# apcamargo/genomad

Hardware: NVIDIA H100
Metric: nn_classification_windows_per_s (higher is better)
Workload: dtype split operands on wgmma (conv: fp16 main pass + two e4m3 correction passes; w_v: 3 fp16 passes), fp32 accumulate; fp32-equivalent (<=1e-4 vs the fp32 oracle, measured ~1e-5)

## Files before the change

genomad_b200/csrc/api.cu:

```cuda
#include <cuda.h>
#include <cuda_runtime.h>
#include <cuda_fp16.h>

#include <algorithm>
#include <cmath>
#include <cstdio>
#include <cstring>
#include <string>
#include <vector>

#include "../../include/gnm.h"
#include "common.cuh"
#include "encode.cuh"
#include "conv_t.cuh"
#include "layer1_wv.cuh"
#include "conv_ref.cuh"
#include "igloo.cuh"
#include "dense.cuh"
#include "logits_tc.cuh"
#include "wv_gather.cuh"
#include "contigs.cuh"
#include "attr.cuh"
#include "neighbours.cuh"
#include "clusters.cuh"
// ... 36 lines not shown
  float* conv1_table = nullptr; float* conv1_triple = nullptr; float* conv1_bias = nullptr;
  uint8_t* wpack[4] = {nullptr, nullptr, nullptr, nullptr};
  float conv_out_scale[2] = {1.f, 1.f};
  float* conv_bias[2] = {nullptr, nullptr};
  float* conv_w32[2] = {nullptr, nullptr};
  float* wv32[2] = {nullptr, nullptr};
  float* ent_w[2] = {nullptr, nullptr}; int32_t* ent_pos[2] = {nullptr, nullptr}; int32_t* slot_of[2] = {nullptr, nullptr};
  float* wbias[2] = {nullptr, nullptr}; float* wqk[2] = {nullptr, nullptr};
  float* d0w = nullptr; float* d0b = nullptr; float* bn0_scale = nullptr; float* bn0_shift = nullptr;
  float* d1w = nullptr; float* d1b = nullptr; float* bn1_scale = nullptr; float* bn1_shift = nullptr;
  float* d2w = nullptr; float* d2b = nullptr;
  float* dwT_hi[2] = {nullptr, nullptr}; float* dwT_lo[2] = {nullptr, nullptr};
  float* hA_hi[2] = {nullptr, nullptr}; float* hA_lo[2] = {nullptr, nullptr};
  CUtensorMap tm_hd_a[2][2]; CUtensorMap tm_hd_b[2][2];
  uint8_t* ybuf[2] = {nullptr, nullptr};
  int ybuf_fp8lo[2] = {0, 0};
  float* q[2] = {nullptr, nullptr};
  float* mpi[2] = {nullptr, nullptr};
  float* mpi_hi[2] = {nullptr, nullptr}; float* mpi_lo[2] = {nullptr, nullptr};
  float* wqkT_hi[2] = {nullptr, nullptr}; float* wqkT_lo[2] = {nullptr, nullptr};
  CUtensorMap tm_lg_a[2][2];
  CUtensorMap tm_lg_b[2][2];
  float* part = nullptr;
  int2* grp[2] = {nullptr, nullptr};
  int32_t* band_gstart[2] = {nullptr, nullptr};
  uint4* wfrag[2] = {nullptr, nullptr};
  float gather_unscale[2] = {1.f, 1.f};
  float wv_out_scale[2] = {1.f, 1.f};
  std::vector<int32_t> band_groups[2];
  int32_t* cta_split = nullptr;
  std::vector<int32_t> split_host[2];
  int split_groups[2] = {-1, -1}, split_grid[2] = {-1, -1};
  float wv_cost_base = 1.f, wv_cost_group = 0.1f;
  int mb_pad = 0;
  CUtensorMap tm_band[2];
  float* logits = nullptr; float* logits_part = nullptr; float* h0 = nullptr; float* h1 = nullptr; float* h2 = nullptr;
  float* scratch32 = nullptr;
  uint8_t* in_stage[2] = {nullptr, nullptr};
  float* out_stage[2] = {nullptr, nullptr};
  float* q_set[2][2] = {{nullptr, nullptr}, {nullptr, nullptr}};
  float* mpi_set[2][2] = {{nullptr, nullptr}, {nullptr, nullptr}};
  float* mpi_hi_set[2][2] = {{nullptr, nullptr}, {nullptr, nullptr}};
  float* mpi_lo_set[2][2] = {{nullptr, nullptr}, {nullptr, nullptr}};
  CUtensorMap tm_lg_a_set[2][2][2];
  int tail_overlap = 1;
  cudaStream_t tail_stream = nullptr;
  cudaEvent_t main_done[2] = {nullptr, nullptr}, tail_done[2] = {nullptr, nullptr};
  cudaStream_t copy_stream = nullptr, compute_stream = nullptr;
  cudaEvent_t in_ready[2] = {nullptr, nullptr}, in_free[2] = {nullptr, nullptr};
  DeviceStatus* status = nullptr;
  CUtensorMap tm_act[2];
  CUtensorMap tm_w[4];
  CUtensorMap tm_w_half[4];
  StageTimer timer;
  std::vector<void*> allocs;
  const uint8_t* attr_route[2] = {nullptr, nullptr};
// ... 114 lines not shown
      pack_stage_f8_pairs(pk, Wk + static_cast<size_t>(tap) * kC * kC, kh, std::ldexp(1.f, d), std::ldexp(1.f, S - 12 - d),
                          std::ldexp(1.f, S - 7 - d));
  return 0;
}

static constexpr int kSplitExpMin = -126, kSplitExpMax = 121;
static bool split_exponent(const float* w, size_t n, int* k) {
  float wmax = 0.f;
  for (size_t i = 0; i < n; ++i) {
    if (!std::isfinite(w[i])) return false;
    wmax = std::max(wmax, std::fabs(w[i]));
  }
  *k = 0;
  if (wmax > 0.f) { int ex; std::frexp(wmax, &ex); *k = std::max(kSplitExpMin, std::min(kSplitExpMax, 14 - ex)); }
  return true;
}

struct PatchPack {
  std::vector<float> ent_w;
  std::vector<int32_t> ent_pos, slot_of;
  std::vector<int2> groups;
  std::vector<int32_t> band_gstart;
  std::vector<uint32_t> frag;
  float unscale = 1.f;
};
static bool pack_patches(const int32_t* patches, const float* w_mult, const float* w_summer, PatchPack& o) {
  std::vector<int> order(static_cast<size_t>(kPatches) * kPatchLen);
  for (size_t i = 0; i < order.size(); ++i) order[i] = static_cast<int>(i);
  std::stable_sort(order.begin(), order.end(), [&](int a, int b) { return patches[a] < patches[b]; });
  o.ent_w.assign(static_cast<size_t>(kGsSlots) * kC, 0.f);
  o.ent_pos.assign(kGsSlots, 0);
  o.slot_of.assign(static_cast<size_t>(kPatches) * kPatchLen, 0);
  std::vector<float>& ent_w = o.ent_w;
  std::vector<int32_t>& ent_pos = o.ent_pos;
  for (size_t slot = 0; slot < order.size(); ++slot) {
    const int e = order[slot], k = e % kPatchLen;
    ent_pos[slot] = patches[e];
    o.slot_of[e] = static_cast<int32_t>(slot);
    for (int c = 0; c < kC; ++c)
      ent_w[slot * kC + c] = (w_mult[static_cast<size_t>(e) * kC + c] * w_summer[k * kC + c]) * (1.f / kActScale);
  }
  int k2;
  if (!split_exponent(ent_w.data(), ent_w.size(), &k2)) return false;
  const float wscale = std::ldexp(1.f, k2);
  o.unscale = std::ldexp(1.f, -k2);
  o.groups.clear();
  o.band_gstart.assign(kNumBands + 1, 0);
  const size_t n_ent = order.size();
  size_t slot = 0;
  for (int b = 0; b < kNumBands; ++b) {
    o.band_gstart[b] = static_cast<int32_t>(o.groups.size());
    while (slot < n_ent && ent_pos[slot] < (b + 1) * kBandRows) {
      size_t run = slot;
      while (run < n_ent && ent_pos[run] == ent_pos[slot] && run - slot < static_cast<size_t>(kWgGroupMax)) ++run;
      o.groups.push_back(make_int2(static_cast<int>(slot), (ent_pos[slot] - b * kBandRows) | (static_cast<int>(run - slot) << 8)));
      slot = run;
    }
  }
  o.band_gstart[kNumBands] = static_cast<int32_t>(o.groups.size());
  if (o.groups.empty()) o.groups.push_back(make_int2(0, 0));
  auto h2 = [](float x, float y) {
    return static_cast<uint32_t>(__half_as_ushort(__float2half_rn(x))) | (static_cast<uint32_t>(__half_as_ushort(__float2half_rn(y))) << 16);
  };
  o.frag.assign(static_cast<size_t>(kGsSlots) * 128, 0u);
  for (size_t e = 0; e < n_ent; ++e)
    for (int kh = 0; kh < 2; ++kh)
      for (int ks = 0; ks < 4; ++ks)
        for (int tig = 0; tig < 4; ++tig) {
          const int k0 = kh * 64 + ks * 16 + 2 * tig;
          const int kk[4] = {k0, k0 + 1, k0 + 8, k0 + 9};
          float hi[4], lo[4];
          for (int i = 0; i < 4; ++i) {
            const float x = ent_w[e * kC + kk[i]] * wscale;
            hi[i] = __half2float(__float2half_rn(x));
            lo[i] = x - hi[i];
          }
          uint32_t* f = &o.frag[(((e * 2 + kh) * 4 + ks) * 4 + tig) * 4];
          f[0] = h2(hi[0], hi[1]); f[1] = h2(hi[2], hi[3]); f[2] = h2(lo[0], lo[1]); f[3] = h2(lo[2], lo[3]);
        }
  return true;
}
extern "C" int gnm_pack_patches(const int32_t* patches, const float* w_mult, const float* w_summer, int32_t* slot_of, int32_t* ent_pos,
                                float* ent_w, int32_t* groups, int* n_groups, int32_t* band_first_group, uint32_t* frag, float* unscale,
                                int* layout) {
  if (layout) { layout[0] = kBandRows; layout[1] = kNumBands; layout[2] = kGsSlots; layout[3] = kWgGroupMax; }
  if (!patches && !w_mult && !w_summer) return 0;
  if (!patches || !w_mult || !w_summer || !n_groups) return fail("gnm_pack_patches: null argument");
  for (int i = 0; i < kPatches * kPatchLen; ++i)
    if (patches[i] < 0 || patches[i] >= kTok) return fail("gnm_pack_patches: patch index out of range");
  PatchPack pk;
  if (!pack_patches(patches, w_mult, w_summer, pk))
    return fail("gnm_pack_patches: folded patch weights w_mult * w_summer / 32 not finite: no fp16 operand split carries them");
  const int real_groups = pk.band_gstart[kNumBands];
  if (groups && *n_groups < real_groups) return fail("gnm_pack_patches: groups buffer too small");
  if (slot_of) std::memcpy(slot_of, pk.slot_of.data(), pk.slot_of.size() * sizeof(int32_t));
  if (ent_pos) std::memcpy(ent_pos, pk.ent_pos.data(), pk.ent_pos.size() * sizeof(int32_t));
  if (ent_w) std::memcpy(ent_w, pk.ent_w.data(), pk.ent_w.size() * sizeof(float));
  if (groups) for (int i = 0; i < real_groups; ++i) { groups[2 * i] = pk.groups[i].x; groups[2 * i + 1] = pk.groups[i].y; }
  *n_groups = real_groups;
  if (band_first_group) std::memcpy(band_first_group, pk.band_gstart.data(), pk.band_gstart.size() * sizeof(int32_t));
  if (frag) std::memcpy(frag, pk.frag.data(), pk.frag.size() * sizeof(uint32_t));
  if (unscale) *unscale = pk.unscale;
  return 0;
}

static void fold_bn(const gnm_bn_weights& b, std::vector<float>& sc, std::vector<float>& sh) {
  sc.resize(kHidden); sh.resize(kHidden);
  for (int i = 0; i < kHidden; ++i) {
// ... 58 lines not shown
      if (dev_upload(h, &h->wpack[L], pk.data(), pk.size())) return 1;
      if (dev_upload(h, &h->conv_w32[L], convw[L], static_cast<size_t>(kTaps) * kC * kC)) return 1;
    }
    for (int s = 0; s < 2; ++s) {
      int e;
      if (!split_exponent(w->igloo[s].w_v, static_cast<size_t>(kC) * kC, &e))
        return fail("gnm_create: IGLOO layer " + std::to_string(s) + ": w_v not finite: no fp16 operand split carries it");
      h->wv_out_scale[s] = std::ldexp(1.f / kActScale, -e);
      std::vector<uint8_t> pk;
      for (int kh = 0; kh < 2; ++kh)
        for (int w_lo = 0; w_lo < 2; ++w_lo) pack_stage_f16(pk, w->igloo[s].w_v, w_lo, kh, std::ldexp(1.f, e));
      if (dev_upload(h, &h->wpack[2 + s], pk.data(), pk.size())) return 1;
    }
    if (dev_upload(h, &h->conv_bias[0], w->conv2_bias, kC)) return 1;
    if (dev_upload(h, &h->conv_bias[1], w->conv3_bias, kC)) return 1;
  }
  for (int s = 0; s < 2; ++s) {
    const gnm_igloo_weights& g = w->igloo[s];
    PatchPack pk;
    if (!pack_patches(g.patches, g.w_mult, g.w_summer, pk))
      return fail("gnm_create: IGLOO layer " + std::to_string(s) +
                  ": folded patch weights w_mult * w_summer / 32 not finite: no fp16 operand split carries them");
    h->gather_unscale[s] = pk.unscale;
    h->band_groups[s].resize(kNumBands);
    for (int b = 0; b < kNumBands; ++b) h->band_groups[s][b] = pk.band_gstart[b + 1] - pk.band_gstart[b];
    if (dev_upload(h, &h->grp[s], pk.groups.data(), pk.groups.size())) return 1;
    if (dev_upload(h, &h->band_gstart[s], pk.band_gstart.data(), pk.band_gstart.size())) return 1;
    if (dev_upload(h, reinterpret_cast<uint32_t**>(&h->wfrag[s]), pk.frag.data(), pk.frag.size())) return 1;
    const std::vector<float>& ent_w = pk.ent_w;
    const std::vector<int32_t>&ent_pos = pk.ent_pos, &slot_of = pk.slot_of;
    if (dev_upload(h, &h->ent_w[s], ent_w.data(), ent_w.size())) return 1;
    if (dev_upload(h, &h->ent_pos[s], ent_pos.data(), ent_pos.size())) return 1;
    if (dev_upload(h, &h->slot_of[s], slot_of.data(), slot_of.size())) return 1;
    if (dev_upload(h, &h->wbias[s], g.w_bias, kPatches)) return 1;
    if (dev_upload(h, &h->wqk[s], g.w_qk, static_cast<size_t>(kPatches) * kPooled)) return 1;
    {
      std::vector<float> thi(static_cast<size_t>(kPooled) * kPatches), tlo(thi.size());
      for (int k = 0; k < kPatches; ++k)
        for (int n = 0; n < kPooled; ++n)
          split_tf32(g.w_qk[static_cast<size_t>(k) * kPooled + n], thi[static_cast<size_t>(n) * kPatches + k],
                     tlo[static_cast<size_t>(n) * kPatches + k]);
      if (dev_upload(h, &h->wqkT_hi[s], thi.data(), thi.size())) return 1;
      if (dev_upload(h, &h->wqkT_lo[s], tlo.data(), tlo.size())) return 1;
    }
    if (dev_upload(h, &h->wv32[s], g.w_v, static_cast<size_t>(kC) * kC)) return 1;
  }
  {
    auto bn = [&](const gnm_bn_weights& b, float** scale, float** shift) -> int {
      std::vector<float> sc, sh;
      fold_bn(b, sc, sh);
      if (dev_upload(h, scale, sc.data(), kHidden)) return 1;
// ... 172 lines not shown
  }
  conv_t_kernel<false><<<grid, kConvThreads, kConvTSmem, st>>>(h->tm_act[in_buf], h->tm_w_half[layer], p);
  return check_launch(h, "conv_t_kernel<false>");
}
static int launch_wv_tc(gnm_handle* h, int s, int buf, int n, cudaStream_t st) {
  ConvTcParams p;
  p.status = h->status;
  p.experiment = 0;
  p.dbg = nullptr;
  p.bias = nullptr; p.y_out = nullptr; p.q_out = h->q[s];
  p.out_scale = h->wv_out_scale[s];
  p.out_fp8 = 0;
  p.n_tiles = n * kUnitsPerWin;
  const int grid = std::min(h->num_sms, p.n_tiles);
  conv_t_kernel<true><<<grid, kConvThreads, kConvTSmem, st>>>(h->tm_act[buf], h->tm_w_half[2 + s], p);
  return check_launch(h, "conv_t_kernel<true>");
}

static int wv_split(gnm_handle* h, int s, int groups, int grid, cudaStream_t st) {
  if (h->split_groups[s] == groups && h->split_grid[s] == grid) return 0;
  std::vector<double> cost(kNumBands);
  double total = 0;
  for (int b = 0; b < kNumBands; ++b) {
    const int per_warp = (h->band_groups[s][b] + kWgWarps - 1) / kWgWarps;
    cost[b] = h->wv_cost_base + h->wv_cost_group * per_warp;
    total += cost[b] * groups;
  }
  std::vector<int32_t>& sp = h->split_host[s];
  sp.assign(h->num_sms + 1, kNumBands * groups);
  sp[0] = 0;
  double acc = 0;
  int c = 1;
  for (int b = 0; b < kNumBands && c < grid; ++b)
    for (int g = 0; g < groups && c < grid; ++g) {
      acc += cost[b];
      if (acc >= total * c / grid) sp[c++] = b * groups + g + 1;
    }
  for (; c <= grid; ++c) sp[c] = kNumBands * groups;
  for (int i = 1; i <= grid; ++i) sp[i] = std::max(sp[i], sp[i - 1]);
  GNM_CUDA(cudaMemcpyAsync(h->cta_split + s * (h->num_sms + 1), sp.data(), (grid + 1) * sizeof(int32_t), cudaMemcpyHostToDevice, st));
  h->split_groups[s] = groups; h->split_grid[s] = grid;
  return 0;
}

static int launch_wv_gather(gnm_handle* h, int s, int buf, int n, cudaStream_t st) {
  WvGatherParams p;
  p.q_out = h->q[s]; p.out_scale = h->wv_out_scale[s];
  p.grp = h->grp[s]; p.band_gstart = h->band_gstart[s]; p.wfrag = h->wfrag[s]; p.gather_unscale = h->gather_unscale[s]; p.part_t = h->part;
  p.n_windows = n;
  p.n_pad = (n + kBandWins - 1) / kBandWins * kBandWins;
  p.groups = p.n_pad / kBandWins;
  p.n_units = kNumBands * p.groups;
  p.status = h->status;
  p.experiment = h->conv_experiment;
  p.dbg = (h->conv_experiment & 512) && s == 1 ? h->conv_dbg : nullptr;
  const int grid = std::min(h->num_sms, p.n_units);
  if (wv_split(h, s, p.groups, grid, st)) return 1;
  p.cta_split = h->cta_split + s * (h->num_sms + 1);
  wv_gather_kernel<<<grid, kWgThreads, kWgSmem, st>>>(h->tm_band[buf], h->tm_w[2 + s], p);
  if (check_launch(h, "wv_gather_kernel")) return 1;
  dim3 fgrid((kPatches + 31) / 32, (n + 31) / 32);
  patch_finish_t_kernel<<<fgrid, 256, 0, st>>>(h->part, h->slot_of[s], h->wbias[s], h->mpi[s], h->mpi_hi[s], h->mpi_lo[s], n, p.n_pad);
  return check_launch(h, "patch_finish_t_kernel");
}

static int ensure_scratch(gnm_handle* h) {
  if (h->scratch32) return 0;
  GNM_CUDA(cudaMalloc(reinterpret_cast<void**>(&h->scratch32), static_cast<size_t>(h->max_batch) * kTok * kC * sizeof(float)));
  return 0;
}

// ... 518 lines not shown
  }
  if (ov.join()) return 1;
  GNM_CUDA(cudaStreamSynchronize(h->compute_stream));
  if (ov.on) GNM_CUDA(cudaStreamSynchronize(h->tail_stream));
  return check_device_status(h);
}
extern "C" int gnm_classify_host(gnm_handle* h, const uint8_t* h_ascii, int n, float* h_probs) {
  return classify_host(h, h_ascii, n, h_probs, nullptr);
}
extern "C" int gnm_embed_host(gnm_handle* h, const uint8_t* h_ascii, int n, float* h_probs, float* d_embed) {
  if (!d_embed && n > 0) return fail("gnm_embed_host: d_embed is null");
  return classify_host(h, h_ascii, n, h_probs, d_embed);
}

extern "C" int gnm_set_option(gnm_handle* h, const char* name, int value) {
  if (!h || !name) return fail("null argument");
  const std::string k(name);
  if (k == "conv_impl") { if (value != 0 && value != 1) return fail("conv_impl must be 0 or 1"); h->conv_impl = value; }
  else if (k == "debug_stop") h->debug_stop = value;
  else if (k == "conv_experiment") h->conv_experiment = value;
  else if (k == "fuse_l1") h->fuse_l1 = value ? 1 : 0;
  else if (k == "fuse_gather") h->fuse_gather = value ? 1 : 0;
  else if (k == "tail_overlap") h->tail_overlap = value ? 1 : 0;
  else if (k == "wv_cost_group") {
    if (value < 0 || value > 10000) return fail("wv_cost_group must be in [0, 10000]");
    h->wv_cost_group = value * 1e-3f; h->split_groups[0] = h->split_groups[1] = -1;
  }
  else if (k == "conv_cluster") { if (value != 1 && value != 2 && value != 4 && value != 8) return fail("conv_cluster must be 1, 2, 4 or 8"); h->conv_cluster = value; }
  else if (k == "profile_stages") { h->profile_stages = value ? 1 : 0; h->timer.names.clear(); }
  else return fail("unknown option: " + k);
  return 0;
}
extern "C" int gnm_get_option(gnm_handle* h, const char* name, int* value) {
  if (!h || !name || !value) return fail("null argument");
  const std::string k(name);
  if (k == "conv_impl") *value = h->conv_impl;
  else if (k == "debug_stop") *value = h->debug_stop;
  else if (k == "profile_stages") *value = h->profile_stages;
  else if (k == "fuse_l1") *value = h->fuse_l1;
  else if (k == "fuse_gather") *value = h->fuse_gather;
  else if (k == "tail_overlap") *value = h->tail_overlap;
  else if (k == "max_batch") *value = h->max_batch;
  else if (k == "num_sms") *value = h->num_sms;
  else return fail("unknown option: " + k);
  return 0;
}
extern "C" long long gnm_kernel_launches(gnm_handle* h) { return h ? h->launches : 0; }

extern "C" int gnm_stage_times(gnm_handle* h, const char** names, float* ms, int* count) {
// ... 822 lines not shown
```

genomad_b200/csrc/wgmma.cuh:

```cuda
#pragma once
#include <stdint.h>

namespace gnm {

__device__ __forceinline__ void wgmma_fence() { asm volatile("wgmma.fence.sync.aligned;" ::: "memory"); }
__device__ __forceinline__ void wgmma_commit() { asm volatile("wgmma.commit_group.sync.aligned;" ::: "memory"); }
template <int kPending> __device__ __forceinline__ void wgmma_wait() {
  asm volatile("wgmma.wait_group.sync.aligned %0;" ::"n"(kPending) : "memory");
}
template <int kN> __device__ __forceinline__ void wgmma_fence_regs(float (&d)[kN]) {
#pragma unroll
  for (int i = 0; i < kN; ++i) asm volatile("" : "+f"(d[i])::"memory");
}

__device__ __forceinline__ uint64_t gmma_desc_sw128(uint32_t saddr) {
  uint64_t d = 0;
  d |= static_cast<uint64_t>((saddr & 0x3FFFF) >> 4);
  d |= static_cast<uint64_t>(1) << 16;
  d |= static_cast<uint64_t>(1024 >> 4) << 32;
  d |= static_cast<uint64_t>(1) << 62;
  return d;
}

#define GNM_ACC8(b) "+f"(d[b]), "+f"(d[b + 1]), "+f"(d[b + 2]), "+f"(d[b + 3]), "+f"(d[b + 4]), "+f"(d[b + 5]), "+f"(d[b + 6]), "+f"(d[b + 7])
__device__ __forceinline__ void wgmma_f16_n48(float (&d)[24], uint64_t da, uint64_t db, uint32_t accumulate) {
  asm volatile("{\n.reg .pred p;\nsetp.ne.b32 p, %26, 0;\n"
               "wgmma.mma_async.sync.aligned.m64n48k16.f32.f16.f16 {%0,%1,%2,%3,%4,%5,%6,%7,%8,%9,%10,%11,%12,%13,%14,%15,%16,%17,%18,%19,%20,%21,%22,%23}, %24,%25,p,1,1,0,0;\n}"
               : GNM_ACC8(0), GNM_ACC8(8), GNM_ACC8(16)
               : "l"(da), "l"(db), "r"(accumulate));
}
__device__ __forceinline__ void wgmma_f16_n192(float (&d)[96], uint64_t da, uint64_t db, uint32_t accumulate) {
  asm volatile("{\n.reg .pred p;\nsetp.ne.b32 p, %98, 0;\n"
               "wgmma.mma_async.sync.aligned.m64n192k16.f32.f16.f16 {%0,%1,%2,%3,%4,%5,%6,%7,%8,%9,%10,%11,%12,%13,%14,%15,%16,%17,%18,%19,%20,%21,%22,%23,%24,%25,%26,%27,%28,%29,%30,%31,%32,%33,%34,%35,%36,%37,%38,%39,%40,%41,%42,%43,%44,%45,%46,%47,%48,%49,%50,%51,%52,%53,%54,%55,%56,%57,%58,%59,%60,%61,%62,%63,%64,%65,%66,%67,%68,%69,%70,%71,%72,%73,%74,%75,%76,%77,%78,%79,%80,%81,%82,%83,%84,%85,%86,%87,%88,%89,%90,%91,%92,%93,%94,%95}, %96,%97,p,1,1,0,0;\n}"
               : GNM_ACC8(0), GNM_ACC8(8), GNM_ACC8(16), GNM_ACC8(24), GNM_ACC8(32), GNM_ACC8(40), GNM_ACC8(48), GNM_ACC8(56), GNM_ACC8(64), GNM_ACC8(72), GNM_ACC8(80), GNM_ACC8(88)
               : "l"(da), "l"(db), "r"(accumulate));
}
__device__ __forceinline__ void wgmma_f16_n256(float (&d)[128], uint64_t da, uint64_t db, uint32_t accumulate) {
  asm volatile("{\n.reg .pred p;\nsetp.ne.b32 p, %130, 0;\n"
               "wgmma.mma_async.sync.aligned.m64n256k16.f32.f16.f16 {%0,%1,%2,%3,%4,%5,%6,%7,%8,%9,%10,%11,%12,%13,%14,%15,%16,%17,%18,%19,%20,%21,%22,%23,%24,%25,%26,%27,%28,%29,%30,%31,%32,%33,%34,%35,%36,%37,%38,%39,%40,%41,%42,%43,%44,%45,%46,%47,%48,%49,%50,%51,%52,%53,%54,%55,%56,%57,%58,%59,%60,%61,%62,%63,%64,%65,%66,%67,%68,%69,%70,%71,%72,%73,%74,%75,%76,%77,%78,%79,%80,%81,%82,%83,%84,%85,%86,%87,%88,%89,%90,%91,%92,%93,%94,%95,%96,%97,%98,%99,%100,%101,%102,%103,%104,%105,%106,%107,%108,%109,%110,%111,%112,%113,%114,%115,%116,%117,%118,%119,%120,%121,%122,%123,%124,%125,%126,%127}, %128,%129,p,1,1,0,0;\n}"
               : GNM_ACC8(0), GNM_ACC8(8), GNM_ACC8(16), GNM_ACC8(24), GNM_ACC8(32), GNM_ACC8(40), GNM_ACC8(48), GNM_ACC8(56), GNM_ACC8(64), GNM_ACC8(72), GNM_ACC8(80), GNM_ACC8(88), GNM_ACC8(96), GNM_ACC8(104), GNM_ACC8(112), GNM_ACC8(120)
               : "l"(da), "l"(db), "r"(accumulate));
}
__device__ __forceinline__ void wgmma_e4m3_n256(float (&d)[128], uint64_t da, uint64_t db, uint32_t accumulate) {
  asm volatile("{\n.reg .pred p;\nsetp.ne.b32 p, %130, 0;\n"
               "wgmma.mma_async.sync.aligned.m64n256k32.f32.e4m3.e4m3 {%0,%1,%2,%3,%4,%5,%6,%7,%8,%9,%10,%11,%12,%13,%14,%15,%16,%17,%18,%19,%20,%21,%22,%23,%24,%25,%26,%27,%28,%29,%30,%31,%32,%33,%34,%35,%36,%37,%38,%39,%40,%41,%42,%43,%44,%45,%46,%47,%48,%49,%50,%51,%52,%53,%54,%55,%56,%57,%58,%59,%60,%61,%62,%63,%64,%65,%66,%67,%68,%69,%70,%71,%72,%73,%74,%75,%76,%77,%78,%79,%80,%81,%82,%83,%84,%85,%86,%87,%88,%89,%90,%91,%92,%93,%94,%95,%96,%97,%98,%99,%100,%101,%102,%103,%104,%105,%106,%107,%108,%109,%110,%111,%112,%113,%114,%115,%116,%117,%118,%119,%120,%121,%122,%123,%124,%125,%126,%127}, %128,%129,p,1,1;\n}"
               : GNM_ACC8(0), GNM_ACC8(8), GNM_ACC8(16), GNM_ACC8(24), GNM_ACC8(32), GNM_ACC8(40), GNM_ACC8(48), GNM_ACC8(56), GNM_ACC8(64), GNM_ACC8(72), GNM_ACC8(80), GNM_ACC8(88), GNM_ACC8(96), GNM_ACC8(104), GNM_ACC8(112), GNM_ACC8(120)
               : "l"(da), "l"(db), "r"(accumulate));
}
__device__ __forceinline__ void wgmma_tf32_n256(float (&d)[128], uint64_t da, uint64_t db, uint32_t accumulate) {
  asm volatile("{\n.reg .pred p;\nsetp.ne.b32 p, %130, 0;\n"
               "wgmma.mma_async.sync.aligned.m64n256k8.f32.tf32.tf32 {%0,%1,%2,%3,%4,%5,%6,%7,%8,%9,%10,%11,%12,%13,%14,%15,%16,%17,%18,%19,%20,%21,%22,%23,%24,%25,%26,%27,%28,%29,%30,%31,%32,%33,%34,%35,%36,%37,%38,%39,%40,%41,%42,%43,%44,%45,%46,%47,%48,%49,%50,%51,%52,%53,%54,%55,%56,%57,%58,%59,%60,%61,%62,%63,%64,%65,%66,%67,%68,%69,%70,%71,%72,%73,%74,%75,%76,%77,%78,%79,%80,%81,%82,%83,%84,%85,%86,%87,%88,%89,%90,%91,%92,%93,%94,%95,%96,%97,%98,%99,%100,%101,%102,%103,%104,%105,%106,%107,%108,%109,%110,%111,%112,%113,%114,%115,%116,%117,%118,%119,%120,%121,%122,%123,%124,%125,%126,%127}, %128,%129,p,1,1;\n}"
               : GNM_ACC8(0), GNM_ACC8(8), GNM_ACC8(16), GNM_ACC8(24), GNM_ACC8(32), GNM_ACC8(40), GNM_ACC8(48), GNM_ACC8(56), GNM_ACC8(64), GNM_ACC8(72), GNM_ACC8(80), GNM_ACC8(88), GNM_ACC8(96), GNM_ACC8(104), GNM_ACC8(112), GNM_ACC8(120)
// ... 12 lines not shown
```

genomad_b200/csrc/wv_gather.cuh:

```cuda
#pragma once
#include <cuda.h>
#include <type_traits>
#include "common.cuh"
#include "conv_t.cuh"
#include "igloo.cuh"

namespace gnm {

constexpr int kBandRows   = 24;
constexpr int kBandWins   = 8;
constexpr int kWgN        = kBandRows * kBandWins;
constexpr int kNumBands   = (kTok + kBandRows - 1) / kBandRows;
constexpr int kWgRegion   = kWgN * 128;
constexpr int kWgBufs     = 6;
constexpr int kWgSlab     = kWgBufs * kWgRegion;
constexpr int kWgWBytes   = kWvStages * kBStage;
constexpr int kWgMmaWarps = 8;
constexpr int kWgWarps    = 7;
constexpr int kWgThreads  = (kWgMmaWarps + kWgWarps + 1) * 32;
constexpr int kWgGroupCap = 4;
constexpr int kWgGroupMax = 4;
constexpr int kWgSmem     = kWgSlab + kWgWBytes + 2048;
static_assert(kWgSmem <= 232448, "wv_gather_kernel exceeds the 227 KB of shared memory a CTA may use");
static_assert(kWgN == 3 * 64 && kBandRows == 3 * kPool && kBandWins == 8, "unit shape: three pool groups of 8 positions x 8 windows");
static_assert(kWgRegion % 1024 == 0, "regions must keep the 1024-byte alignment of the 128-byte swizzle");

struct WvGatherParams {
  float* q_out;
  float out_scale;
  const int2* grp;
  const int32_t* band_gstart;
  const uint4* wfrag;
  float gather_unscale;
  float* part_t;
  int n_windows, n_pad;
  int groups;
  int n_units;
  const int32_t* cta_split;
  int experiment;
  long long* dbg;
  DeviceStatus* status;
};

__device__ __forceinline__ uint2 ldg_frag(const uint2* p) {
  uint2 v;
  asm volatile("ld.global.nc.L1::evict_last.v2.u32 {%0, %1}, [%2];" : "=r"(v.x), "=r"(v.y) : "l"(p));
  return v;
}
__device__ __forceinline__ void ldsm_x4(uint32_t saddr, uint32_t (&a)[4]) {
  asm volatile("ldmatrix.sync.aligned.m8n8.x4.shared.b16 {%0, %1, %2, %3}, [%4];"
               : "=r"(a[0]), "=r"(a[1]), "=r"(a[2]), "=r"(a[3]) : "r"(saddr));
}
__device__ __forceinline__ void mma_16816(float (&d)[4], const uint32_t (&a)[4], uint32_t b0, uint32_t b1) {
  asm volatile("mma.sync.aligned.m16n8k16.row.col.f32.f16.f16.f32 {%0, %1, %2, %3}, {%4, %5, %6, %7}, {%8, %9}, {%0, %1, %2, %3};"
               : "+f"(d[0]), "+f"(d[1]), "+f"(d[2]), "+f"(d[3]) : "r"(a[0]), "r"(a[1]), "r"(a[2]), "r"(a[3]), "r"(b0), "r"(b1));
}

__global__ void __launch_bounds__(kWgThreads, 1)
wv_gather_kernel(const __grid_constant__ CUtensorMap tm_band, const __grid_constant__ CUtensorMap tm_w, const WvGatherParams p) {
  extern __shared__ uint8_t smem_raw[];
  uint8_t* smem = reinterpret_cast<uint8_t*>((reinterpret_cast<uintptr_t>(smem_raw) + 1023) & ~uintptr_t(1023));
  uint8_t* s_a = smem;
  uint8_t* s_w = smem + kWgSlab;
  uint64_t* bars = reinterpret_cast<uint64_t*>(s_w + kWgWBytes);
  uint64_t* a_full = bars;
  uint64_t* a_empty = bars + 8;
  uint64_t* w_full = bars + 16;

  const int warp = __shfl_sync(0xffffffffu, static_cast<int>(threadIdx.x) >> 5, 0);
  const int lane = threadIdx.x & 31;
  constexpr int kProducerWarp = kWgMmaWarps + kWgWarps;
  const int u_begin = p.cta_split[blockIdx.x], u_end = p.cta_split[blockIdx.x + 1];

  if (warp == kProducerWarp && elect_one()) {
    tma_prefetch_desc(&tm_band);
    tma_prefetch_desc(&tm_w);
    for (int i = 0; i < kWgBufs; ++i) { mbar_init(&a_full[i], 1); mbar_init(&a_empty[i], kWgMmaWarps + kWgWarps); }
    mbar_init(w_full, 1);
    fence_barrier_init();
  }
  __syncthreads();

  if (warp == kProducerWarp) {
    if (elect_one()) {
      mbar_arrive_expect_tx(w_full, kWgWBytes);
      for (int q = 0; q < kWvStages; ++q) tma_load_2d_hint(s_w + q * kBStage, &tm_w, w_full, 0, q * 128, l2_policy_evict_last());
      const uint64_t pol = l2_policy_evict_first();
      uint32_t phases = 0;
      int b0 = 0;
      long long c_wait_empty = 0;
      for (int unit = u_begin; unit < u_end; ++unit) {
        const int band = unit / p.groups;
        const int w0 = (unit - band * p.groups) * kBandWins;
#pragma unroll
        for (int k = 0; k < 4; ++k) {
          int b = b0 + k; if (b >= kWgBufs) b -= kWgBufs;
          const long long tq = clock64();
          mbar_wait(&a_empty[b], ((phases >> b) & 1) ^ 1, p.status, 500 + b);
          c_wait_empty += clock64() - tq;
          phases ^= 1u << b;
// ... 55 lines not shown
      const int w0 = (unit - band * p.groups) * kBandWins;
#pragma unroll
      for (int pg = 0; pg < kBandRows / kPool; ++pg) {
        const int gg = band * (kBandRows / kPool) + pg;
        if (gg < kPooled && !(p.experiment & 128)) {
#pragma unroll
          for (int h = 0; h < 2; ++h)
#pragma unroll
            for (int e = 0; e < 2; ++e) {
              float m = d[32 * pg + 2 * h + e];
#pragma unroll
              for (int i = 1; i < kPool; ++i) m = fmaxf(m, d[32 * pg + 4 * i + 2 * h + e]);
              const int w = w0 + win0 + e;
              if (w < p.n_windows) p.q_out[(static_cast<size_t>(w) * kPooled + gg) * kC + ch0 + 8 * h] = m * oscale;
            }
        }
      }
      __syncwarp();
      if (lane == 0) { mbar_arrive(&a_empty[buf(2)]); mbar_arrive(&a_empty[buf(3)]); }
      t_epi += clock() - t_epi0;
      b0 += 4; if (b0 >= kWgBufs) b0 -= kWgBufs;
    }
    if (p.dbg && warp == 0 && lane == 0) { long long* o = p.dbg + blockIdx.x * 8; o[3] = t_mma; o[4] = w_a; o[6] = t_epi; }
  } else {
    const int gw = warp - kWgMmaWarps;
    const float gscale = p.gather_unscale;
    const int lm_plane = (lane >> 3) & 1, lm_chunk = lane >> 4, lm_win = lane & 7;
    const int gid = lane >> 2, tig = lane & 3;
    const uint32_t slab = smem_u32(s_a);
    int it = 0;
    uint32_t phases = 0;
    int b0 = 0;
    long long c_wait_full = 0, c_gather = 0, tq = 0;
    const long long t_begin = clock64();
    int cur_band = -1, g_first = 0, g_cnt = 0, n_mine = 0;
    int my_e0[kWgGroupCap] = {}, my_meta[kWgGroupCap] = {};
    bool fast = true;
    struct GroupFrag { uint2 b[4]; uint32_t a[4][4]; };
    auto load_group = [&](int e0, int meta, int kh, uint32_t hi_base, uint32_t lo_base, GroupFrag& f) {
      const int row = meta & 31, ne = meta >> 8;
      const uint2* wf = reinterpret_cast<const uint2*>(p.wfrag) + ((static_cast<size_t>(e0 + (gid >> 1)) * 2 + kh) * 16 + tig) * 2 + (gid & 1);
#pragma unroll
      for (int ks = 0; ks < 4; ++ks) f.b[ks] = ((gid >> 1) < ne && !(p.experiment & 1024)) ? ldg_frag(wf + ks * 8) : make_uint2(0u, 0u);
      const uint32_t rb = (lm_plane ? lo_base : hi_base) + row * (kBandWins * 128) + lm_win * 128;
#pragma unroll
      for (int ks = 0; ks < 4; ++ks) {
        if (p.experiment & 2048) { f.a[ks][0] = f.a[ks][1] = f.a[ks][2] = f.a[ks][3] = rb; continue; }
        ldsm_x4(rb + (((ks * 2 + lm_chunk) ^ lm_win) << 4), f.a[ks]);
      }
    };
    auto mma_group = [&](const GroupFrag& f) -> float {
      float d[4][4];
#pragma unroll
      for (int ks = 0; ks < 4; ++ks) d[ks][0] = d[ks][1] = d[ks][2] = d[ks][3] = 0.f;
      if (p.experiment & 256) {
#pragma unroll
        for (int ks = 0; ks < 4; ++ks) asm volatile("" :: "r"(f.a[ks][0] | f.a[ks][1] | f.a[ks][2] | f.a[ks][3] | f.b[ks].x | f.b[ks].y));
      } else {
#pragma unroll
        for (int ks = 0; ks < 4; ++ks) mma_16816(d[ks], f.a[ks], f.b[ks].x, f.b[ks].y);
      }
      float v = 0.f;
#pragma unroll
      for (int ks = 0; ks < 4; ++ks) v += (d[ks][0] + d[ks][2]) + (d[ks][1] + d[ks][3]);
      return v * gscale;
    };
    for (int unit = u_begin; unit < u_end; ++unit, ++it) {
      const int band = unit / p.groups;
      const int w0 = (unit - band * p.groups) * kBandWins;
      if (band != cur_band) {
        cur_band = band;
        g_first = p.band_gstart[band];
        g_cnt = (p.experiment & 32) ? 0 : p.band_gstart[band + 1] - g_first;
        fast = g_cnt <= kWgWarps * kWgGroupCap;
        n_mine = 0;
#pragma unroll
        for (int i = 0; i < kWgGroupCap; ++i) {
          const int gi = gw + i * kWgWarps;
          if (fast && gi < g_cnt) { const int2 m = p.grp[g_first + gi]; my_e0[i] = m.x; my_meta[i] = m.y; n_mine = i + 1; }
        }
      }
      float c0[kWgGroupCap];
#pragma unroll 1
      for (int kh = 0; kh < 2; ++kh) {
        int bh = b0 + 2 * kh; if (bh >= kWgBufs) bh -= kWgBufs;
        int bl = b0 + 2 * kh + 1; if (bl >= kWgBufs) bl -= kWgBufs;
        const uint32_t ph_h = (phases >> bh) & 1, ph_l = (phases >> bl) & 1;
        phases ^= (1u << bh) | (1u << bl);
        const uint32_t hi_base = slab + bh * kWgRegion, lo_base = slab + bl * kWgRegion;
        if (p.dbg) tq = clock64();
        mbar_wait(&a_full[bh], ph_h, p.status, 550 + bh);
        mbar_wait(&a_full[bl], ph_l, p.status, 560 + bl);
        if (p.dbg) { const long long t = clock64(); c_wait_full += t - tq; tq = t; }
        if (fast) {
          auto finish = [&](int i, float v) {
            if (kh == 0) c0[i] = v;
            else if (tig < (my_meta[i] >> 8) && !(p.experiment & 64))
              p.part_t[static_cast<size_t>(my_e0[i] + tig) * p.n_pad + w0 + gid] = c0[i] + v;
          };
#pragma unroll
          for (int i = 0; i < kWgGroupCap; i += 2)
            if (i < n_mine) {
              GroupFrag f0, f1;
              load_group(my_e0[i], my_meta[i], kh, hi_base, lo_base, f0);
              if (i + 1 < n_mine) {
                load_group(my_e0[i + 1], my_meta[i + 1], kh, hi_base, lo_base, f1);
                finish(i, mma_group(f0));
                finish(i + 1, mma_group(f1));
              } else {
                finish(i, mma_group(f0));
              }
            }
        } else {
#pragma unroll 1
          for (int gi = gw; gi < g_cnt; gi += kWgWarps) {
            const int2 m = p.grp[g_first + gi];
            GroupFrag f;
            load_group(m.x, m.y, kh, hi_base, lo_base, f);
            const float v = mma_group(f);
            if (tig < (m.y >> 8)) {
              float* gp = p.part_t + static_cast<size_t>(m.x + tig) * p.n_pad + w0 + gid;
              *gp = kh == 0 ? v : *gp + v;
            }
          }
        }
        __syncwarp();
        if (lane == 0) { mbar_arrive(&a_empty[bh]); mbar_arrive(&a_empty[bl]); }
        if (p.dbg) c_gather += clock64() - tq;
      }
      b0 += 4; if (b0 >= kWgBufs) b0 -= kWgBufs;
    }
    if (p.dbg && warp == kWgMmaWarps && lane == 0) {
      long long* d = p.dbg + blockIdx.x * 8;
      d[0] = clock64() - t_begin; d[1] = c_wait_full; d[2] = c_gather; d[5] = it;
    }
  }
}

__global__ void __launch_bounds__(256)
patch_finish_t_kernel(const float* __restrict__ part_t, const int32_t* __restrict__ slot_of, const float* __restrict__ w_bias,
                      float* __restrict__ mpi, float* __restrict__ mpi_hi, float* __restrict__ mpi_lo, int n_windows, int n_pad) {
  __shared__ float tile[32][33];
  const int p0 = blockIdx.x * 32, w0 = blockIdx.y * 32;
  const int tx = threadIdx.x & 31, ty = threadIdx.x >> 5;
  for (int pp = ty; pp < 32; pp += 8) {
    const int pch = p0 + pp, w = w0 + tx;
    float v = 0.f;
    if (pch < kPatches && w < n_windows) {
      const int4 s4 = *reinterpret_cast<const int4*>(slot_of + pch * 4);
      v = (((part_t[static_cast<size_t>(s4.x) * n_pad + w] + part_t[static_cast<size_t>(s4.y) * n_pad + w]) +
            part_t[static_cast<size_t>(s4.z) * n_pad + w]) + part_t[static_cast<size_t>(s4.w) * n_pad + w]) + w_bias[pch];
    }
    tile[pp][tx] = v;
  }
  __syncthreads();
  for (int ww = ty; ww < 32; ww += 8) {
    const int pch = p0 + tx, w = w0 + ww;
// ... 13 lines not shown
```

Measured before the change: 76680.

## Replace per-warp mma.sync entry gather with 64-row wgmma tiles from registers

Patch entries are repacked on the host into 64-row tiles per band, with pre-swizzled fp16 hi/lo A fragments. The gather warps become a single warpgroup of four entry warps issuing register-sourced m64n64k16 wgmma against the swizzled activation slab, replacing seven warps of ldmatrix plus mma.sync per group. Results are picked out per pool position with selects and written as float2. This cuts instruction and ldmatrix overhead and shrinks the CTA from 16 to 12 active warps. In exchange, every tile does a full 64-row wgmma even when a band has only a few entries, so padding adds wasted work, and the load-balancing cost model now counts tiles.

```diff
diff --git a/genomad_b200/csrc/api.cu b/genomad_b200/csrc/api.cu
--- a/genomad_b200/csrc/api.cu
+++ b/genomad_b200/csrc/api.cu
@@ -82,16 +82,16 @@
   CUtensorMap tm_lg_a[2][2];
   CUtensorMap tm_lg_b[2][2];
   float* part = nullptr;
-  int2* grp[2] = {nullptr, nullptr};
-  int32_t* band_gstart[2] = {nullptr, nullptr};
-  uint4* wfrag[2] = {nullptr, nullptr};
+  uint32_t* ent_afrag[2] = {nullptr, nullptr};
+  int32_t* ent_meta[2] = {nullptr, nullptr};
+  int32_t* band_tile[2] = {nullptr, nullptr};
   float gather_unscale[2] = {1.f, 1.f};
   float wv_out_scale[2] = {1.f, 1.f};
-  std::vector<int32_t> band_groups[2];
+  std::vector<int32_t> band_tiles[2];
   int32_t* cta_split = nullptr;
   std::vector<int32_t> split_host[2];
   int split_groups[2] = {-1, -1}, split_grid[2] = {-1, -1};
-  float wv_cost_base = 1.f, wv_cost_group = 0.1f;
+  float wv_cost_base = 1.f, wv_cost_tile = 1.f;
   int mb_pad = 0;
   CUtensorMap tm_band[2];
   float* logits = nullptr; float* logits_part = nullptr; float* h0 = nullptr; float* h1 = nullptr; float* h2 = nullptr;
@@ -252,8 +252,12 @@
   std::vector<int2> groups;
   std::vector<int32_t> band_gstart;
   std::vector<uint32_t> frag;
+  std::vector<uint32_t> afrag;
+  std::vector<int32_t> tile_meta;
+  std::vector<int32_t> band_tile;
   float unscale = 1.f;
 };
+static constexpr int kHookGroupMax = 4;
 static bool pack_patches(const int32_t* patches, const float* w_mult, const float* w_summer, PatchPack& o) {
   std::vector<int> order(static_cast<size_t>(kPatches) * kPatchLen);
   for (size_t i = 0; i < order.size(); ++i) order[i] = static_cast<int>(i);
@@ -282,7 +286,7 @@
     o.band_gstart[b] = static_cast<int32_t>(o.groups.size());
     while (slot < n_ent && ent_pos[slot] < (b + 1) * kBandRows) {
       size_t run = slot;
-      while (run < n_ent && ent_pos[run] == ent_pos[slot] && run - slot < static_cast<size_t>(kWgGroupMax)) ++run;
+      while (run < n_ent && ent_pos[run] == ent_pos[slot] && run - slot < static_cast<size_t>(kHookGroupMax)) ++run;
       o.groups.push_back(make_int2(static_cast<int>(slot), (ent_pos[slot] - b * kBandRows) | (static_cast<int>(run - slot) << 8)));
       slot = run;
     }
@@ -308,12 +312,48 @@
           uint32_t* f = &o.frag[(((e * 2 + kh) * 4 + ks) * 4 + tig) * 4];
           f[0] = h2(hi[0], hi[1]); f[1] = h2(hi[2], hi[3]); f[2] = h2(lo[0], lo[1]); f[3] = h2(lo[2], lo[3]);
         }
+  o.band_tile.assign(kNumBands + 1, 0);
+  o.afrag.clear();
+  o.tile_meta.clear();
+  slot = 0;
+  for (int b = 0; b < kNumBands; ++b) {
+    const size_t t0 = o.tile_meta.size() / kWgTileRows;
+    o.band_tile[b] = static_cast<int32_t>(t0);
+    const size_t first = slot;
+    while (slot < n_ent && ent_pos[slot] < (b + 1) * kBandRows) ++slot;
+    const size_t n_tiles = std::max<size_t>(1, (slot - first + kWgTileRows - 1) / kWgTileRows);
+    o.tile_meta.resize((t0 + n_tiles) * kWgTileRows, -1);
+    o.afrag.resize((t0 + n_tiles) * kWgTileWords, 0u);
+    for (size_t t = 0; t < n_tiles; ++t) {
+      auto w_at = [&](int r, int k, int part) {
+        const size_t e = first + t * kWgTileRows + r;
+        if (e >= slot) return 0.f;
+        const float x = ent_w[e * kC + k] * wscale, hi = __half2float(__float2half_rn(x));
+        return part ? x - hi : hi;
+      };
+      for (int r = 0; r < kWgTileRows; ++r) {
+        const size_t e = first + t * kWgTileRows + r;
+        if (e < slot) o.tile_meta[(t0 + t) * kWgTileRows + r] = static_cast<int32_t>(e) | ((ent_pos[e] - b * kBandRows) << 16);
+      }
+      uint32_t* tw = o.afrag.data() + (t0 + t) * kWgTileWords;
+      for (int kh = 0; kh < 2; ++kh)
+        for (int ks = 0; ks < 4; ++ks)
+          for (int part = 0; part < 2; ++part)
+            for (int th = 0; th < 128; ++th) {
+              const int r = 16 * (th >> 5) + ((th & 31) >> 2), k0 = 64 * kh + 16 * ks + 2 * (th & 3);
+              const int rr[4] = {r, r + 8, r, r + 8}, kk[4] = {k0, k0, k0 + 8, k0 + 8};
+              uint32_t* f = tw + (((kh * 4 + ks) * 2 + part) * 128 + th) * 4;
+              for (int i = 0; i < 4; ++i) f[i] = h2(w_at(rr[i], kk[i], part), w_at(rr[i], kk[i] + 1, part));
+            }
+    }
+  }
+  o.band_tile[kNumBands] = static_cast<int32_t>(o.tile_meta.size() / kWgTileRows);
   return true;
 }
 extern "C" int gnm_pack_patches(const int32_t* patches, const float* w_mult, const float* w_summer, int32_t* slot_of, int32_t* ent_pos,
                                 float* ent_w, int32_t* groups, int* n_groups, int32_t* band_first_group, uint32_t* frag, float* unscale,
                                 int* layout) {
-  if (layout) { layout[0] = kBandRows; layout[1] = kNumBands; layout[2] = kGsSlots; layout[3] = kWgGroupMax; }
+  if (layout) { layout[0] = kBandRows; layout[1] = kNumBands; layout[2] = kGsSlots; layout[3] = kHookGroupMax; }
   if (!patches && !w_mult && !w_summer) return 0;
   if (!patches || !w_mult || !w_summer || !n_groups) return fail("gnm_pack_patches: null argument");
   for (int i = 0; i < kPatches * kPatchLen; ++i)
@@ -418,11 +458,11 @@
       return fail("gnm_create: IGLOO layer " + std::to_string(s) +
                   ": folded patch weights w_mult * w_summer / 32 not finite: no fp16 operand split carries them");
     h->gather_unscale[s] = pk.unscale;
-    h->band_groups[s].resize(kNumBands);
-    for (int b = 0; b < kNumBands; ++b) h->band_groups[s][b] = pk.band_gstart[b + 1] - pk.band_gstart[b];
-    if (dev_upload(h, &h->grp[s], pk.groups.data(), pk.groups.size())) return 1;
-    if (dev_upload(h, &h->band_gstart[s], pk.band_gstart.data(), pk.band_gstart.size())) return 1;
-    if (dev_upload(h, reinterpret_cast<uint32_t**>(&h->wfrag[s]), pk.frag.data(), pk.frag.size())) return 1;
+    h->band_tiles[s].resize(kNumBands);
+    for (int b = 0; b < kNumBands; ++b) h->band_tiles[s][b] = pk.band_tile[b + 1] - pk.band_tile[b];
+    if (dev_upload(h, &h->ent_afrag[s], pk.afrag.data(), pk.afrag.size())) return 1;
+    if (dev_upload(h, &h->ent_meta[s], pk.tile_meta.data(), pk.tile_meta.size())) return 1;
+    if (dev_upload(h, &h->band_tile[s], pk.band_tile.data(), pk.band_tile.size())) return 1;
     const std::vector<float>& ent_w = pk.ent_w;
     const std::vector<int32_t>&ent_pos = pk.ent_pos, &slot_of = pk.slot_of;
     if (dev_upload(h, &h->ent_w[s], ent_w.data(), ent_w.size())) return 1;
@@ -641,8 +681,7 @@
   std::vector<double> cost(kNumBands);
   double total = 0;
   for (int b = 0; b < kNumBands; ++b) {
-    const int per_warp = (h->band_groups[s][b] + kWgWarps - 1) / kWgWarps;
-    cost[b] = h->wv_cost_base + h->wv_cost_group * per_warp;
+    cost[b] = h->wv_cost_base + h->wv_cost_tile * (h->band_tiles[s][b] - 1);
     total += cost[b] * groups;
   }
   std::vector<int32_t>& sp = h->split_host[s];
@@ -665,7 +704,8 @@
 static int launch_wv_gather(gnm_handle* h, int s, int buf, int n, cudaStream_t st) {
   WvGatherParams p;
   p.q_out = h->q[s]; p.out_scale = h->wv_out_scale[s];
-  p.grp = h->grp[s]; p.band_gstart = h->band_gstart[s]; p.wfrag = h->wfrag[s]; p.gather_unscale = h->gather_unscale[s]; p.part_t = h->part;
+  p.ent_afrag = reinterpret_cast<const uint4*>(h->ent_afrag[s]); p.ent_meta = h->ent_meta[s]; p.band_tile = h->band_tile[s];
+  p.gather_unscale = h->gather_unscale[s]; p.part_t = h->part;
   p.n_windows = n;
   p.n_pad = (n + kBandWins - 1) / kBandWins * kBandWins;
   p.groups = p.n_pad / kBandWins;
@@ -1230,9 +1270,9 @@
   else if (k == "fuse_l1") h->fuse_l1 = value ? 1 : 0;
   else if (k == "fuse_gather") h->fuse_gather = value ? 1 : 0;
   else if (k == "tail_overlap") h->tail_overlap = value ? 1 : 0;
-  else if (k == "wv_cost_group") {
-    if (value < 0 || value > 10000) return fail("wv_cost_group must be in [0, 10000]");
-    h->wv_cost_group = value * 1e-3f; h->split_groups[0] = h->split_groups[1] = -1;
+  else if (k == "wv_cost_tile") {
+    if (value < 0 || value > 10000) return fail("wv_cost_tile must be in [0, 10000]");
+    h->wv_cost_tile = value * 1e-3f; h->split_groups[0] = h->split_groups[1] = -1;
   }
   else if (k == "conv_cluster") { if (value != 1 && value != 2 && value != 4 && value != 8) return fail("conv_cluster must be 1, 2, 4 or 8"); h->conv_cluster = value; }
   else if (k == "profile_stages") { h->profile_stages = value ? 1 : 0; h->timer.names.clear(); }
diff --git a/genomad_b200/csrc/wgmma.cuh b/genomad_b200/csrc/wgmma.cuh
--- a/genomad_b200/csrc/wgmma.cuh
+++ b/genomad_b200/csrc/wgmma.cuh
@@ -28,6 +28,12 @@
                "wgmma.mma_async.sync.aligned.m64n48k16.f32.f16.f16 {%0,%1,%2,%3,%4,%5,%6,%7,%8,%9,%10,%11,%12,%13,%14,%15,%16,%17,%18,%19,%20,%21,%22,%23}, %24,%25,p,1,1,0,0;\n}"
                : GNM_ACC8(0), GNM_ACC8(8), GNM_ACC8(16)
                : "l"(da), "l"(db), "r"(accumulate));
+}
+__device__ __forceinline__ void wgmma_f16_rs_n64(float (&d)[32], const uint4& a, uint64_t db, uint32_t accumulate) {
+  asm volatile("{\n.reg .pred p;\nsetp.ne.b32 p, %37, 0;\n"
+               "wgmma.mma_async.sync.aligned.m64n64k16.f32.f16.f16 {%0,%1,%2,%3,%4,%5,%6,%7,%8,%9,%10,%11,%12,%13,%14,%15,%16,%17,%18,%19,%20,%21,%22,%23,%24,%25,%26,%27,%28,%29,%30,%31}, {%32,%33,%34,%35}, %36,p,1,1,0;\n}"
+               : GNM_ACC8(0), GNM_ACC8(8), GNM_ACC8(16), GNM_ACC8(24)
+               : "r"(a.x), "r"(a.y), "r"(a.z), "r"(a.w), "l"(db), "r"(accumulate));
 }
 __device__ __forceinline__ void wgmma_f16_n192(float (&d)[96], uint64_t da, uint64_t db, uint32_t accumulate) {
   asm volatile("{\n.reg .pred p;\nsetp.ne.b32 p, %98, 0;\n"
diff --git a/genomad_b200/csrc/wv_gather.cuh b/genomad_b200/csrc/wv_gather.cuh
--- a/genomad_b200/csrc/wv_gather.cuh
+++ b/genomad_b200/csrc/wv_gather.cuh
@@ -16,10 +16,10 @@
 constexpr int kWgSlab     = kWgBufs * kWgRegion;
 constexpr int kWgWBytes   = kWvStages * kBStage;
 constexpr int kWgMmaWarps = 8;
-constexpr int kWgWarps    = 7;
-constexpr int kWgThreads  = (kWgMmaWarps + kWgWarps + 1) * 32;
-constexpr int kWgGroupCap = 4;
-constexpr int kWgGroupMax = 4;
+constexpr int kWgEntryWarps = 4;
+constexpr int kWgThreads  = 16 * 32;
+constexpr int kWgTileRows = 64;
+constexpr int kWgTileWords = kWgTileRows * 128 * 2 / 2;
 constexpr int kWgSmem     = kWgSlab + kWgWBytes + 2048;
 static_assert(kWgSmem <= 232448, "wv_gather_kernel exceeds the 227 KB of shared memory a CTA may use");
 static_assert(kWgN == 3 * 64 && kBandRows == 3 * kPool && kBandWins == 8, "unit shape: three pool groups of 8 positions x 8 windows");
@@ -28,9 +28,9 @@
 struct WvGatherParams {
   float* q_out;
   float out_scale;
-  const int2* grp;
-  const int32_t* band_gstart;
-  const uint4* wfrag;
+  const uint4* ent_afrag;
+  const int32_t* ent_meta;
+  const int32_t* band_tile;
   float gather_unscale;
   float* part_t;
   int n_windows, n_pad;
@@ -42,20 +42,6 @@
   DeviceStatus* status;
 };
 
-__device__ __forceinline__ uint2 ldg_frag(const uint2* p) {
-  uint2 v;
-  asm volatile("ld.global.nc.L1::evict_last.v2.u32 {%0, %1}, [%2];" : "=r"(v.x), "=r"(v.y) : "l"(p));
-  return v;
-}
-__device__ __forceinline__ void ldsm_x4(uint32_t saddr, uint32_t (&a)[4]) {
-  asm volatile("ldmatrix.sync.aligned.m8n8.x4.shared.b16 {%0, %1, %2, %3}, [%4];"
-               : "=r"(a[0]), "=r"(a[1]), "=r"(a[2]), "=r"(a[3]) : "r"(saddr));
-}
-__device__ __forceinline__ void mma_16816(float (&d)[4], const uint32_t (&a)[4], uint32_t b0, uint32_t b1) {
-  asm volatile("mma.sync.aligned.m16n8k16.row.col.f32.f16.f16.f32 {%0, %1, %2, %3}, {%4, %5, %6, %7}, {%8, %9}, {%0, %1, %2, %3};"
-               : "+f"(d[0]), "+f"(d[1]), "+f"(d[2]), "+f"(d[3]) : "r"(a[0]), "r"(a[1]), "r"(a[2]), "r"(a[3]), "r"(b0), "r"(b1));
-}
-
 __global__ void __launch_bounds__(kWgThreads, 1)
 wv_gather_kernel(const __grid_constant__ CUtensorMap tm_band, const __grid_constant__ CUtensorMap tm_w, const WvGatherParams p) {
   extern __shared__ uint8_t smem_raw[];
@@ -69,13 +55,13 @@
 
   const int warp = __shfl_sync(0xffffffffu, static_cast<int>(threadIdx.x) >> 5, 0);
   const int lane = threadIdx.x & 31;
-  constexpr int kProducerWarp = kWgMmaWarps + kWgWarps;
+  constexpr int kProducerWarp = 15;
   const int u_begin = p.cta_split[blockIdx.x], u_end = p.cta_split[blockIdx.x + 1];
 
   if (warp == kProducerWarp && elect_one()) {
     tma_prefetch_desc(&tm_band);
     tma_prefetch_desc(&tm_w);
-    for (int i = 0; i < kWgBufs; ++i) { mbar_init(&a_full[i], 1); mbar_init(&a_empty[i], kWgMmaWarps + kWgWarps); }
+    for (int i = 0; i < kWgBufs; ++i) { mbar_init(&a_full[i], 1); mbar_init(&a_empty[i], kWgMmaWarps + kWgEntryWarps); }
     mbar_init(w_full, 1);
     fence_barrier_init();
   }
@@ -177,117 +163,104 @@
       b0 += 4; if (b0 >= kWgBufs) b0 -= kWgBufs;
     }
     if (p.dbg && warp == 0 && lane == 0) { long long* o = p.dbg + blockIdx.x * 8; o[3] = t_mma; o[4] = w_a; o[6] = t_epi; }
-  } else {
-    const int gw = warp - kWgMmaWarps;
-    const float gscale = p.gather_unscale;
-    const int lm_plane = (lane >> 3) & 1, lm_chunk = lane >> 4, lm_win = lane & 7;
-    const int gid = lane >> 2, tig = lane & 3;
-    const uint32_t slab = smem_u32(s_a);
-    int it = 0;
+  } else if (warp < kWgMmaWarps + kWgEntryWarps) {
+    const int wq = warp & 3;
+    const uint32_t a_base = smem_u32(s_a);
+    const int m0 = wq * 16 + (lane >> 2);
+    const int win0 = 2 * (lane & 3);
+    const int tid = threadIdx.x - kWgMmaWarps * 32;
+    const bool work = !(p.experiment & 32);
     uint32_t phases = 0;
-    int b0 = 0;
-    long long c_wait_full = 0, c_gather = 0, tq = 0;
-    const long long t_begin = clock64();
-    int cur_band = -1, g_first = 0, g_cnt = 0, n_mine = 0;
-    int my_e0[kWgGroupCap] = {}, my_meta[kWgGroupCap] = {};
-    bool fast = true;
-    struct GroupFrag { uint2 b[4]; uint32_t a[4][4]; };
-    auto load_group = [&](int e0, int meta, int kh, uint32_t hi_base, uint32_t lo_base, GroupFrag& f) {
-      const int row = meta & 31, ne = meta >> 8;
-      const uint2* wf = reinterpret_cast<const uint2*>(p.wfrag) + ((static_cast<size_t>(e0 + (gid >> 1)) * 2 + kh) * 16 + tig) * 2 + (gid & 1);
-#pragma unroll
-      for (int ks = 0; ks < 4; ++ks) f.b[ks] = ((gid >> 1) < ne && !(p.experiment & 1024)) ? ldg_frag(wf + ks * 8) : make_uint2(0u, 0u);
-      const uint32_t rb = (lm_plane ? lo_base : hi_base) + row * (kBandWins * 128) + lm_win * 128;
-#pragma unroll
-      for (int ks = 0; ks < 4; ++ks) {
-        if (p.experiment & 2048) { f.a[ks][0] = f.a[ks][1] = f.a[ks][2] = f.a[ks][3] = rb; continue; }
-        ldsm_x4(rb + (((ks * 2 + lm_chunk) ^ lm_win) << 4), f.a[ks]);
-      }
-    };
-    auto mma_group = [&](const GroupFrag& f) -> float {
-      float d[4][4];
-#pragma unroll
-      for (int ks = 0; ks < 4; ++ks) d[ks][0] = d[ks][1] = d[ks][2] = d[ks][3] = 0.f;
-      if (p.experiment & 256) {
-#pragma unroll
-        for (int ks = 0; ks < 4; ++ks) asm volatile("" :: "r"(f.a[ks][0] | f.a[ks][1] | f.a[ks][2] | f.a[ks][3] | f.b[ks].x | f.b[ks].y));
-      } else {
-#pragma unroll
-        for (int ks = 0; ks < 4; ++ks) mma_16816(d[ks], f.a[ks], f.b[ks].x, f.b[ks].y);
-      }
-      float v = 0.f;
-#pragma unroll
-      for (int ks = 0; ks < 4; ++ks) v += (d[ks][0] + d[ks][2]) + (d[ks][1] + d[ks][3]);
-      return v * gscale;
-    };
-    for (int unit = u_begin; unit < u_end; ++unit, ++it) {
+    int b0 = 0, loaded = -1;
+    uint32_t w_a = 0, t_mma = 0, t_epi = 0;
+    uint4 a[2][4][2];
+    float d[32];
+    for (int unit = u_begin; unit < u_end; ++unit) {
+      auto buf = [&](int k) { const int b = b0 + k; return b >= kWgBufs ? b - kWgBufs : b; };
       const int band = unit / p.groups;
       const int w0 = (unit - band * p.groups) * kBandWins;
-      if (band != cur_band) {
-        cur_band = band;
-        g_first = p.band_gstart[band];
-        g_cnt = (p.experiment & 32) ? 0 : p.band_gstart[band + 1] - g_first;
-        fast = g_cnt <= kWgWarps * kWgGroupCap;
-        n_mine = 0;
-#pragma unroll
-        for (int i = 0; i < kWgGroupCap; ++i) {
-          const int gi = gw + i * kWgWarps;
-          if (fast && gi < g_cnt) { const int2 m = p.grp[g_first + gi]; my_e0[i] = m.x; my_meta[i] = m.y; n_mine = i + 1; }
-        }
-      }
-      float c0[kWgGroupCap];
+      const int t_first = p.band_tile[band], t_last = p.band_tile[band + 1] - 1;
+      const uint32_t t_unit = clock();
 #pragma unroll 1
-      for (int kh = 0; kh < 2; ++kh) {
-        int bh = b0 + 2 * kh; if (bh >= kWgBufs) bh -= kWgBufs;
-        int bl = b0 + 2 * kh + 1; if (bl >= kWgBufs) bl -= kWgBufs;
-        const uint32_t ph_h = (phases >> bh) & 1, ph_l = (phases >> bl) & 1;
-        phases ^= (1u << bh) | (1u << bl);
-        const uint32_t hi_base = slab + bh * kWgRegion, lo_base = slab + bl * kWgRegion;
-        if (p.dbg) tq = clock64();
-        mbar_wait(&a_full[bh], ph_h, p.status, 550 + bh);
-        mbar_wait(&a_full[bl], ph_l, p.status, 560 + bl);
-        if (p.dbg) { const long long t = clock64(); c_wait_full += t - tq; tq = t; }
-        if (fast) {
-          auto finish = [&](int i, float v) {
-            if (kh == 0) c0[i] = v;
-            else if (tig < (my_meta[i] >> 8) && !(p.experiment & 64))
-              p.part_t[static_cast<size_t>(my_e0[i] + tig) * p.n_pad + w0 + gid] = c0[i] + v;
-          };
-#pragma unroll
-          for (int i = 0; i < kWgGroupCap; i += 2)
-            if (i < n_mine) {
-              GroupFrag f0, f1;
-              load_group(my_e0[i], my_meta[i], kh, hi_base, lo_base, f0);
-              if (i + 1 < n_mine) {
-                load_group(my_e0[i + 1], my_meta[i + 1], kh, hi_base, lo_base, f1);
-                finish(i, mma_group(f0));
-                finish(i + 1, mma_group(f1));
-              } else {
-                finish(i, mma_group(f0));
+      for (int t = t_first; t <= t_last; ++t) {
+        if (t != loaded) {
+          const uint4* src = p.ent_afrag + static_cast<size_t>(t) * (kWgTileWords / 4) + tid;
+#pragma unroll
+          for (int kh = 0; kh < 2; ++kh)
+#pragma unroll
+            for (int kk = 0; kk < 4; ++kk)
+#pragma unroll
+              for (int hl = 0; hl < 2; ++hl) a[kh][kk][hl] = __ldg(src + ((kh * 4 + kk) * 2 + hl) * 128);
+          loaded = t;
+        }
+        const int meta0 = p.ent_meta[t * kWgTileRows + m0], meta1 = p.ent_meta[t * kWgTileRows + m0 + 8];
+#pragma unroll 1
+        for (int c = 0; c < kBandRows / kPool; ++c) {
+#pragma unroll
+          for (int kh = 0; kh < 2; ++kh) {
+            if (t == t_first && c == 0) {
+#pragma unroll
+              for (int r = 0; r < 2; ++r) {
+                const int b = buf(2 * kh + r);
+                const uint32_t tq = clock();
+                mbar_wait(&a_full[b], (phases >> b) & 1, p.status, 550 + b);
+                w_a += clock() - tq;
+                phases ^= 1u << b;
               }
             }
-        } else {
-#pragma unroll 1
-          for (int gi = gw; gi < g_cnt; gi += kWgWarps) {
-            const int2 m = p.grp[g_first + gi];
-            GroupFrag f;
-            load_group(m.x, m.y, kh, hi_base, lo_base, f);
-            const float v = mma_group(f);
-            if (tig < (m.y >> 8)) {
-              float* gp = p.part_t + static_cast<size_t>(m.x + tig) * p.n_pad + w0 + gid;
-              *gp = kh == 0 ? v : *gp + v;
+            if (work) {
+              const uint64_t yh = gmma_desc_sw128(a_base + buf(2 * kh) * kWgRegion + c * 64 * 128);
+              const uint64_t yl = gmma_desc_sw128(a_base + buf(2 * kh + 1) * kWgRegion + c * 64 * 128);
+              wgmma_fence();
+#pragma unroll
+              for (int kk = 0; kk < 4; ++kk) {
+                wgmma_f16_rs_n64(d, a[kh][kk][0], yh + kk * 2, (kh == 0 && kk == 0) ? 0u : 1u);
+                wgmma_f16_rs_n64(d, a[kh][kk][0], yl + kk * 2, 1u);
+              }
+#pragma unroll
+              for (int kk = 0; kk < 4; ++kk) wgmma_f16_rs_n64(d, a[kh][kk][1], yh + kk * 2, 1u);
+              wgmma_commit();
             }
           }
-        }
-        __syncwarp();
-        if (lane == 0) { mbar_arrive(&a_empty[bh]); mbar_arrive(&a_empty[bl]); }
-        if (p.dbg) c_gather += clock64() - tq;
-      }
+          const bool last = t == t_last && c == kBandRows / kPool - 1;
+          wgmma_wait<1>();
+          __syncwarp();
+          if (lane == 0 && last) { mbar_arrive(&a_empty[buf(0)]); mbar_arrive(&a_empty[buf(1)]); }
+          wgmma_wait<0>();
+          wgmma_fence_regs(d);
+          __syncwarp();
+          if (lane == 0 && last) { mbar_arrive(&a_empty[buf(2)]); mbar_arrive(&a_empty[buf(3)]); }
+          const uint32_t t_epi0 = clock();
+          const int r0 = (meta0 >> 16) - 8 * c, r1 = (meta1 >> 16) - 8 * c;
+          float v00 = 0.f, v01 = 0.f, v10 = 0.f, v11 = 0.f;
+#pragma unroll
+          for (int j = 0; j < kPool; ++j) {
+            v00 = j == r0 ? d[4 * j] : v00;
+            v01 = j == r0 ? d[4 * j + 1] : v01;
+            v10 = j == r1 ? d[4 * j + 2] : v10;
+            v11 = j == r1 ? d[4 * j + 3] : v11;
+          }
+          const int w = w0 + win0;
+          if (work && !(p.experiment & 64) && w < p.n_windows) {
+#pragma unroll
+            for (int h = 0; h < 2; ++h) {
+              const int meta = h ? meta1 : meta0, r = h ? r1 : r0;
+              if (meta < 0 || r < 0 || r >= kPool) continue;
+              float* dst = p.part_t + static_cast<size_t>(meta & 0xffff) * p.n_pad + w;
+              const float x = (h ? v10 : v00) * p.gather_unscale, y = (h ? v11 : v01) * p.gather_unscale;
+              if (w + 1 < p.n_windows) *reinterpret_cast<float2*>(dst) = make_float2(x, y);
+              else dst[0] = x;
+            }
+          }
+          t_epi += clock() - t_epi0;
+        }
+      }
+      t_mma += clock() - t_unit;
       b0 += 4; if (b0 >= kWgBufs) b0 -= kWgBufs;
     }
     if (p.dbg && warp == kWgMmaWarps && lane == 0) {
-      long long* d = p.dbg + blockIdx.x * 8;
-      d[0] = clock64() - t_begin; d[1] = c_wait_full; d[2] = c_gather; d[5] = it;
+      long long* o = p.dbg + blockIdx.x * 8;
+      o[0] = t_mma; o[1] = w_a; o[2] = t_epi; o[5] = u_end - u_begin;
     }
   }
 }
```

New measurement: 76130 (median of 6 runs). No clear change (-0.7%).
